# AI-Application-and-Integration-Lab/RDPN6D

Measured on AMD Instinct MI355X. Metric: RGB-D crops/sec (fwd+PnP) at 256x256, higher is better.
Workload: dtype f32

## Files before the change

include/rdpn6d.h:

```cpp
#ifndef RDPN6D_H
#define RDPN6D_H

#ifdef __cplusplus
extern "C" {
#endif

#define RDPN6D_OK 0
#define RDPN6D_EINVAL -1
#define RDPN6D_EHIP -2
#define RDPN6D_ENOMEM -3

const char* rdpn6d_last_error(void);
int rdpn6d_version(void);
int rdpn6d_device_count(void);

void farthest_point_sampling(float* pts, int* idxs, int pn, int sn);
void farthest_point_sampling_init_center(float* pts, int* idxs, int pn, int sn);
int rdpn6d_fps_host(const float* pts, int* idxs, int pn, int sn, int start);
int rdpn6d_fps_device(const float* d_pts, const int* d_offsets, int nobj, int max_pn, int sn, int start,
                      int* d_idxs, float* d_mindist, void* stream);
long long rdpn6d_fps_workspace_bytes(int nobj);
int rdpn6d_fps_device_ws(const float* d_pts, const int* d_offsets, int nobj, int max_pn, int sn, int start, int* d_idxs,
                         float* d_mindist, void* workspace, long long workspace_bytes, void* stream);

// ... 206 lines not shown
int rdpn6d_dense_glue_backward_f32(const float* head, int head_cs, const float* coord2d, const float* fps, const int* argmax,
                                   const float* dpnp, int pnp_cs, int B, int HW, int K, int mask_attention,
                                   const float* minmax, float* dhead, float* datt_scratch, void* stream);
int rdpn6d_dense_losses_mt_f32(const float* head, int head_cs, const float* gt_xyz, const float* mask_visib, const float* mask_trunc,
                               const long long* gt_region, int B, int HW, int K, float xyz_lw, float mask_lw, float region_lw,
                               int mask_type, float* dhead, float* losses, double* scratch, void* stream);
int rdpn6d_dense_glue_backward_mt_f32(const float* head, int head_cs, const float* coord2d, const float* fps, const int* argmax,
                                      const float* dpnp, int pnp_cs, int B, int HW, int K, int mask_attention, int mask_type,
                                      const float* minmax, float* dhead, float* datt_scratch, void* stream);
int rdpn6d_pose_train_f32(const float* rt, int rt_stride, const float* roi_cams, const float* roi_centers,
                          const float* roi_whs, const float* resize_ratios, const float* roi_extents, const float* gt_rot,
                          const float* gt_trans_ratio, const float* points, int npts, int B, int is_allo, float pm_lw,
                          int pm_norm_by_extent, float centroid_lw, float z_lw, float* rot, float* trans, float* d_rt,
                          float* losses, float* scratch, void* stream);
int rdpn6d_pose_train_sym_f32(const float* rt, int rt_stride, const float* roi_cams, const float* roi_centers,
                              const float* roi_whs, const float* resize_ratios, const float* roi_extents,
                              const float* gt_rot, const float* gt_trans_ratio, const float* points, int npts, int B,
                              int is_allo, float pm_lw, int pm_norm_by_extent, float centroid_lw, float z_lw,
                              const float* sym_rots, const int* sym_counts, int ksym, float* gt_rot_used, float* rot,
                              float* trans, float* d_rt, float* losses, float* scratch, void* stream);
int rdpn6d_train_vis_scalars_f32(const float* rot, const float* trans, const float* gt_rot, const float* gt_trans, const float* rt,
                                 int rt_stride, const float* gt_trans_ratio, int B, float* out17, void* stream);
int rdpn6d_ranger_step_f32(float* param, const float* grad, float* exp_avg, float* exp_avg_sq, float* slow, const void* work,
                           int nwork, const long long* row_off, const int* row_len, int nrows, float* row_mean, float beta1,
                           float beta2, float eps, float neg_step_lr, float wd_lr, int rectified, int lookahead, float alpha,
                           void* stream);
int rdpn6d_ranger_step_scaled_f32(float* param, const float* grad, float* exp_avg, float* exp_avg_sq, float* slow, const void* work,
                                  int nwork, const long long* row_off, const int* row_len, int nrows, float* row_mean, float beta1,
                                  float beta2, float eps, float neg_step_lr, float wd_lr, int rectified, int lookahead, float alpha,
                                  float inv_scale, const int* found_inf, void* stream);
int rdpn6d_grad_nonfinite_f32(const float* grad, long long n, int* flag, void* stream);
int rdpn6d_act_backward_f32(float* dy, const float* y, long long n, float slope, void* stream);
int rdpn6d_transpose_rc_f32(const float* x, int B, int R, int C, float* y, void* stream);
int rdpn6d_rgb_to_nhwc4_f32(const float* x, int B, int xc, int R, float* y, void* stream);
int rdpn6d_stem_im2col_f32(const float* x, int B, int xc, int R, float* out, void* stream);
int rdpn6d_stem_rowpatch_f32(const float* x, int B, int xc, int R, float* out, void* stream);

typedef struct {
    const float* src;
    float* dst;
    void* dst_bf16;
    const int* operm;
    const int* iperm;
    long long so, si, start;
    int O, T, I, dT, dIpad;
    int toff[9];
} rdpn6d_repack_desc;
int rdpn6d_repack_f32(const rdpn6d_repack_desc* table_dev, const int* blk_desc_dev, const long long* blk_off_dev, int nblocks,
                      void* stream);

int rdpn6d_bn_train_stats_bf16(const void* x, long long M, int C, int cs, int co, float eps, float momentum, float* mean,
                               float* invstd, float* running_mean, float* running_var, double* scratch, void* stream);
int rdpn6d_bn_apply_bf16(const void* x, int xcs, int xco, const float* mean, const float* invstd, const float* gamma,
                         const float* beta, const void* res, int rcs, int rco, void* y, int ycs, int yco, long long M, int C,
                         int relu, void* stream);
int rdpn6d_bn_backward_bf16(const void* x, int xcs, int xco, const void* dy, int dcs, int dco, const void* y, int ycs, int yco,
                            const float* mean, const float* invstd, const float* gamma, float* dgamma, float* dbeta, void* dx,
                            int xgcs, int xgco, void* dres, int rcs, int rco, long long M, int C, int relu, double* scratch,
                            void* stream);
int rdpn6d_bn_relu_backward_bf16(const void* x, int xcs, int xco, const void* dy, int dcs, int dco, const float* mean,
                                 const float* invstd, const float* gamma, const float* beta, float* dgamma, float* dbeta, void* dx,
                                 int xgcs, int xgco, long long M, int C, double* scratch, void* stream);
int rdpn6d_channel_sum_bf16(const void* x, long long M, int C, int cs, int co, float* out, int accumulate, double* scratch,
                            void* stream);
int rdpn6d_maxpool3x3s2_backward_bf16(const void* x, const void* dy, int B, int H, int W, int C, void* dx, void* stream);
int rdpn6d_upsample_bilinear_backward_bf16(const void* dy, int B, int H, int W, int C, int factor, void* dx, void* stream);
// ... 103 lines not shown
```

rdpn6d_amd/_lib.py:

```python
import ctypes
import os

HERE = os.path.dirname(os.path.abspath(__file__))
LIB_PATH = os.environ.get("RDPN6D_LIB") or os.path.join(HERE, "librdpn6d_hip.so")

_ll = ctypes.c_longlong
c_float_p = ctypes.c_void_p
c_int_p = ctypes.c_void_p
_vp, _i, _f, _u = ctypes.c_void_p, ctypes.c_int, ctypes.c_float, ctypes.c_uint


class ConvDesc(ctypes.Structure):

    _fields_ = [
        ("x", _vp), ("w", _vp), ("scale", _vp), ("shift", _vp), ("res", _vp), ("y", _vp),
        ("B", _i), ("H", _i), ("W", _i), ("Cin", _i), ("in_cs", _i), ("in_co", _i), ("Ho", _i), ("Wo", _i),
        ("stride", _i), ("ntaps", _i), ("dy", _i * 9), ("dx", _i * 9), ("N", _i), ("Npad", _i), ("OH", _i), ("OW", _i),
        ("osy", _i), ("osx", _i), ("ooy", _i), ("oox", _i), ("out_cs", _i), ("out_co", _i), ("res_cs", _i),
        ("res_co", _i), ("act", _i), ("slope", _f),
    ]


SIGNATURES = {
    "rdpn6d_last_error": (ctypes.c_char_p, []),
# ... 65 lines not shown
    "rdpn6d_groupnorm_relu_train_f32": (_i, [_vp, _vp, _i, _i, _i, _i, _vp, _vp, _vp, _vp]),
    "rdpn6d_groupnorm_relu_backward_f32": (_i, [_vp, _vp, _vp, _vp, _vp, _vp, _vp, _vp, _vp, _vp, _i, _i, _i, _i, _vp]),
    "rdpn6d_wgrad_scratch_floats": (_ll, [_i, _i, _i, _i, _i, _i]),
    "rdpn6d_wgrad_f32": (_i, [_vp, _i, _i, _i, _vp, _i, _i, _i, _i, _i, _i, _i, _i, _i, _i, _vp, _vp, _vp, _vp, _vp]),
    "rdpn6d_wgrad_bf16": (_i, [_vp, _i, _i, _i, _i, _vp, _i, _i, _i, _i, _i, _i, _i, _i, _i, _i, _i, _vp, _vp, _vp, _vp, _vp]),
    "rdpn6d_wgrad_f32_strided": (_i, [_vp, _i, _i, _i, _vp, _i, _i, _i, _i, _i, _i, _i, _i, _i, _i, _vp, _vp, _vp, _ll, _ll, _ll, _i, _i,
                                      _vp, _vp]),
    "rdpn6d_wgrad_bf16_strided": (_i, [_vp, _i, _i, _i, _i, _vp, _i, _i, _i, _i, _i, _i, _i, _i, _i, _i, _i, _vp, _vp, _vp, _ll, _ll, _ll,
                                       _i, _i, _vp, _vp]),
    "rdpn6d_wgrad_group_scratch_floats": (_ll, [_i, _i, _i, _i, _i, _i, _i]),
    "rdpn6d_wgrad_bf16_group": (_i, [_i, _vp, _i, _i, _i, _i, _vp, _i, _i, _i, _i, _i, _i, _i, _i, _i, _i, _i, _vp, _vp, _vp, _ll, _ll, _ll,
                                     _i, _i, _vp, _ll, _vp]),
    "rdpn6d_wgrad_bf16x3_strided": (_i, [_vp, _ll, _i, _i, _i, _i, _vp, _ll, _i, _i, _i, _i, _i, _i, _i, _i, _i, _i, _i, _vp, _vp, _vp,
                                         _ll, _ll, _ll, _i, _i, _vp, _vp]),
    "rdpn6d_maxpool3x3s2_backward_f32": (_i, [_vp, _vp, _i, _i, _i, _i, _vp, _vp]),
    "rdpn6d_upsample_bilinear_backward_f32": (_i, [_vp, _i, _i, _i, _i, _i, _vp, _vp]),
    "rdpn6d_global_max_concat_backward_f32": (_i, [_vp, _vp, _i, _i, _i, _i, _vp, _vp]),
    "rdpn6d_dense_losses_f32": (_i, [_vp, _i, _vp, _vp, _vp, _vp, _i, _i, _i, _f, _f, _f, _vp, _vp, _vp, _vp]),
    "rdpn6d_dense_glue_backward_f32": (_i, [_vp, _i, _vp, _vp, _vp, _vp, _i, _i, _i, _i, _i, _vp, _vp, _vp, _vp]),
    "rdpn6d_dense_losses_mt_f32": (_i, [_vp, _i, _vp, _vp, _vp, _vp, _i, _i, _i, _f, _f, _f, _i, _vp, _vp, _vp, _vp]),
    "rdpn6d_dense_glue_backward_mt_f32": (_i, [_vp, _i, _vp, _vp, _vp, _vp, _i, _i, _i, _i, _i, _i, _vp, _vp, _vp, _vp]),
    "rdpn6d_pose_train_f32": (_i, [_vp, _i, _vp, _vp, _vp, _vp, _vp, _vp, _vp, _vp, _i, _i, _i, _f, _i, _f, _f, _vp, _vp, _vp,
                                   _vp, _vp, _vp]),
    "rdpn6d_pose_train_sym_f32": (_i, [_vp, _i, _vp, _vp, _vp, _vp, _vp, _vp, _vp, _vp, _i, _i, _i, _f, _i, _f, _f, _vp, _vp, _i,
                                       _vp, _vp, _vp, _vp, _vp, _vp, _vp]),
    "rdpn6d_ranger_step_f32": (_i, [_vp, _vp, _vp, _vp, _vp, _vp, _i, _vp, _vp, _i, _vp, _f, _f, _f, _f, _f, _i, _i, _f, _vp]),
    "rdpn6d_ranger_step_scaled_f32": (_i, [_vp, _vp, _vp, _vp, _vp, _vp, _i, _vp, _vp, _i, _vp, _f, _f, _f, _f, _f, _i, _i, _f, _f, _vp, _vp]),
    "rdpn6d_grad_nonfinite_f32": (_i, [_vp, _ll, _vp, _vp]),
    "rdpn6d_region_targets_f32": (_i, [_vp, _vp, _vp, _vp, _i, _i, _i, _vp, _vp, _vp]),
    "rdpn6d_pose_errors_f64": (_i, [_vp, _vp, _vp, _i, _i, _i, _vp, _vp, _vp]),
    "rdpn6d_crop_builder_f32": (_i, [_vp, _vp, _i, _i, _i, _vp, _vp, _vp, _vp, _vp, _i, _i, _vp, _vp, _vp]),
    "rdpn6d_act_backward_f32": (_i, [_vp, _vp, _ll, _f, _vp]),
    "rdpn6d_transpose_rc_f32": (_i, [_vp, _i, _i, _i, _vp, _vp]),
    "rdpn6d_train_vis_scalars_f32": (_i, [_vp, _vp, _vp, _vp, _vp, _i, _vp, _i, _vp, _vp]),
    "rdpn6d_rgb_to_nhwc4_f32": (_i, [_vp, _i, _i, _i, _vp, _vp]),
    "rdpn6d_stem_im2col_f32": (_i, [_vp, _i, _i, _i, _vp, _vp]),
    "rdpn6d_stem_rowpatch_f32": (_i, [_vp, _i, _i, _i, _vp, _vp]),
    "rdpn6d_stem_conv7x7_raw_bf16": (_i, [_vp, _i, _i, _i, _vp, _vp, _vp]),
    "rdpn6d_bn_train_stats_bf16": (_i, [_vp, _ll, _i, _i, _i, _f, _f, _vp, _vp, _vp, _vp, _vp, _vp]),
    "rdpn6d_bn_apply_bf16": (_i, [_vp, _i, _i, _vp, _vp, _vp, _vp, _vp, _i, _i, _vp, _i, _i, _ll, _i, _i, _vp]),
    "rdpn6d_bn_backward_bf16": (_i, [_vp, _i, _i, _vp, _i, _i, _vp, _i, _i, _vp, _vp, _vp, _vp, _vp, _vp, _i, _i, _vp, _i, _i,
                                     _ll, _i, _i, _vp, _vp]),
    "rdpn6d_bn_relu_backward_bf16": (_i, [_vp, _i, _i, _vp, _i, _i, _vp, _vp, _vp, _vp, _vp, _vp, _vp, _i, _i, _ll, _i, _vp, _vp]),
    "rdpn6d_channel_sum_bf16": (_i, [_vp, _ll, _i, _i, _i, _vp, _i, _vp, _vp]),
    "rdpn6d_maxpool3x3s2_backward_bf16": (_i, [_vp, _vp, _i, _i, _i, _i, _vp, _vp]),
    "rdpn6d_upsample_bilinear_backward_bf16": (_i, [_vp, _i, _i, _i, _i, _i, _vp, _vp]),
    "rdpn6d_global_max_concat_backward_bf16": (_i, [_vp, _vp, _i, _i, _i, _i, _vp, _vp]),
    "rdpn6d_stem_im2col_bf16": (_i, [_vp, _i, _i, _i, _vp, _vp]),
    "rdpn6d_stem_rowpatch_bf16": (_i, [_vp, _i, _i, _i, _vp, _vp]),
    "rdpn6d_repack_f32": (_i, [_vp, _vp, _vp, _i, _vp]),
    "rdpn6d_split_h2": (_i, [_vp, _i, _i, _i, _vp, _ll, _vp, _vp]),
    "rdpn6d_conv_h2_kernel_for": (_i, [_vp]),
    "rdpn6d_conv2d_h2": (_i, [_vp, _vp, _vp, _vp, _vp]),
    "rdpn6d_upsample_bilinear_h2": (_i, [_vp, _i, _i, _i, _i, _i, _vp, _vp, _vp]),
    "rdpn6d_xyz_subsample_h2": (_i, [_vp, _i, _i, _i, _i, _vp, _i, _i, _vp, _vp]),
    "rdpn6d_stem_pool_h2": (_i, [_vp, _i, _i, _i, _vp, _vp, _vp, _vp, _vp, _vp]),
    "rdpn6d_stem_pool_h2_ex": (_i, [_vp, _i, _i, _i, _vp, _vp, _vp, _vp, _i, _vp, _vp]),
    "rdpn6d_stem_pack_h2": (_i, [_vp, _vp, _vp, _vp]),
    "rdpn6d_global_max_concat_h2": (_i, [_vp, _i, _i, _i, _i, _vp]),
    "rdpn6d_upsample_bilinear_h2_ex": (_i, [_vp, _i, _i, _i, _i, _i, _vp, _i, _i, _i, _vp, _vp]),
    "rdpn6d_global_max_h2": (_i, [_vp, _i, _i, _i, _i, _vp, _vp]),
    "rdpn6d_convt3x3s2_const_bias_f32": (_i, [_vp, _vp, _i, _i, _vp, _vp]),
    "rdpn6d_conv2d_h2_cb": (_i, [_vp, _vp, _vp, _vp, _vp, _vp]),
    "rdpn6d_conv2d_h2_ws": (_i, [_vp, _vp, _vp, _vp, _vp, _vp, ctypes.c_longlong, _vp]),
    "rdpn6d_conv_h2_fuse1x1_ok": (_i, [ctypes.POINTER(ConvDesc)]),
    "rdpn6d_conv2d_h2_fuse1x1": (_i, [ctypes.POINTER(ConvDesc), _vp, _vp, _vp, _vp, _vp, _vp, _vp, _i, _i, _vp]),
# ... 50 lines not shown
```

rdpn6d_amd/build.py:

```python
import os
import subprocess
import sys

HERE = os.path.dirname(os.path.abspath(__file__))
CSRC = os.path.join(HERE, "csrc")
LIB = os.path.join(HERE, "librdpn6d_hip.so")
SOURCES = ["api.cpp", "conv_igemm.hip", "conv_igemm_bf16.hip", "conv_igemm_bf16_8ph.hip", "conv_igemm_bf16_pp.hip", "conv_igemm_bf16x3.hip", "conv_igemm_bf16x3_tile.hip", "conv_igemm_h2.hip", "conv_igemm_h2_pp.hip", "pointwise.hip", "pointwise_bf16.hip", "pointwise_h2.hip", "fps.hip", "ransac.hip", "train_norm.hip", "train_wgrad.hip", "train_misc.hip", "ranger.hip", "targets_eval.hip", "crop_builder.hip", "pnp.hip"]
NO_CONTRACT = {"fps.hip", "ransac.hip", "targets_eval.hip", "crop_builder.hip", "pnp.hip"}
FLAGS = ["--offload-arch=gfx950", "-O3", "-std=c++17", "-fPIC", "-Wall", "-Wno-unused-function"]
LP_SOURCES = ["conv_igemm_bf16.hip", "conv_igemm_bf16_8ph.hip", "conv_igemm_bf16_pp.hip", "pointwise_bf16.hip", "pointwise.hip", "train_norm.hip", "train_misc.hip",
              "train_wgrad.hip"]
LP_EXTRA_RENAMES = {"rdpn6d_repack_f32": "rdpn6d_repack_fp16"}
if os.environ.get("RDPN6D_PROBE"):
    FLAGS.append("-DRDPN6D_PROBE")


def _stale():
    if not os.path.exists(LIB):
        return True
    t = os.path.getmtime(LIB)
    deps = [os.path.join(CSRC, f) for f in os.listdir(CSRC)] + [os.path.join(HERE, "..", "include", "rdpn6d.h")]
    return any(os.path.getmtime(d) > t for d in deps)


def build(force=False, verbose=True):
    if not force and not _stale():
        return LIB
    hipcc = os.environ.get("HIPCC", "/opt/rocm/bin/hipcc")
    objs = []
    os.makedirs(os.path.join(HERE, "build"), exist_ok=True)
    procs = []
    for src in SOURCES:
        obj = os.path.join(HERE, "build", src + ".o")
        objs.append(obj)
        extra = ["-ffp-contract=off"] if src in NO_CONTRACT else []
        cmd = [hipcc] + FLAGS + extra + ["-c", os.path.join(CSRC, src), "-o", obj]
        procs.append((src, subprocess.Popen(cmd, stdout=subprocess.PIPE, stderr=subprocess.STDOUT, text=True)))
    lp_objs = []
    for src in LP_SOURCES:
        obj = os.path.join(HERE, "build", "fp16_" + src + ".o")
# ... 40 lines not shown
```

rdpn6d_amd/config.py:

```python
import ast
import copy
import os


class ConfigDict(dict):

    def __init__(self, *a, **k):
        super().__init__()
        for key, v in dict(*a, **k).items():
            self[key] = v

    def __setitem__(self, k, v):
        super().__setitem__(k, _wrap(v))

    def __getattr__(self, k):
        try:
            return self[k]
        except KeyError as e:
            raise AttributeError(f"config has no key '{k}'") from e

    def __setattr__(self, k, v):
        self[k] = v

    def update(self, *a, **k):
# ... 82 lines not shown
            WEIGHTS="",
            PIXEL_MEAN=[0.0, 0.0, 0.0],
            PIXEL_STD=[255.0, 255.0, 255.0],
            CDPN=dict(
                NAME="GDRN",
                TASK="rot",
                USE_MTL=False,
                BACKBONE=dict(PRETRAINED="", ARCH="resnet", NUM_LAYERS=34, INPUT_CHANNEL=3, INPUT_RES=256,
                              OUTPUT_RES=64, FREEZE=False),
                ROT_HEAD=dict(
                    FREEZE=False, ROT_CONCAT=False, XYZ_BIN=64, NUM_LAYERS=3, NUM_FILTERS=256, CONV_KERNEL_SIZE=3,
                    NORM="BN", NUM_GN_GROUPS=32, OUT_CONV_KERNEL_SIZE=1, NUM_CLASSES=num_classes,
                    ROT_CLASS_AWARE=False, XYZ_LOSS_TYPE="L1", XYZ_LOSS_MASK_GT="visib", XYZ_LW=1.0,
                    MASK_CLASS_AWARE=False, MASK_LOSS_TYPE="L1", MASK_LOSS_GT="trunc", MASK_LW=1.0,
                    MASK_THR_TEST=0.5, NUM_REGIONS=num_regions, REGION_CLASS_AWARE=False, REGION_LOSS_TYPE="CE",
                    REGION_LOSS_MASK_GT="visib", REGION_LW=1.0,
                ),
                PNP_NET=dict(
                    FREEZE=False, R_ONLY=False, LR_MULT=1.0,
                    PNP_HEAD_CFG=dict(type="ConvPnPNet", norm="GN", num_gn_groups=32, drop_prob=0.0),
                    WITH_2D_COORD=True, REGION_ATTENTION=True, MASK_ATTENTION=mask_attention,
                    TRANS_WITH_BOX_INFO="none", ROT_TYPE="allo_rot6d", TRANS_TYPE="centroid_z", Z_TYPE="REL",
                    NUM_PM_POINTS=3000, PM_LOSS_TYPE="L1", PM_SMOOTH_L1_BETA=1.0, PM_LOSS_SYM=False,
                    PM_NORM_BY_EXTENT=True, PM_R_ONLY=True, PM_DISENTANGLE_T=False, PM_DISENTANGLE_Z=False,
                    PM_T_USE_POINTS=False, PM_LW=1.0, ROT_LOSS_TYPE="angular", ROT_LW=0.0,
                    CENTROID_LOSS_TYPE="L1", CENTROID_LW=1.0, Z_LOSS_TYPE="L1", Z_LW=1.0, TRANS_LOSS_TYPE="L1",
                    TRANS_LOSS_DISENTANGLE=True, TRANS_LW=0.0, BIND_LOSS_TYPE="L1", BIND_LW=0.0,
                ),
                TRANS_HEAD=dict(ENABLED=False, FREEZE=True, LR_MULT=1.0, NUM_LAYERS=3, NUM_FILTERS=256, NORM="BN",
                                NUM_GN_GROUPS=32, CONV_KERNEL_SIZE=3, OUT_CHANNEL=3, TRANS_TYPE="centroid_z",
                                Z_TYPE="REL"),
            ),
        ),
        SOLVER=dict(IMS_PER_BATCH=24, BASE_LR=1e-4, BF16X3=True, GROUP_WGRAD=True, OPTIMIZER_CFG=dict(type="Ranger", lr=1e-4, weight_decay=0),
                    WEIGHT_DECAY=0.0, AMP=dict(ENABLED=False, DTYPE="bf16")),
        INPUT=dict(FORMAT="BGR", DZI_PAD_SCALE=1.5),
        TRAIN=dict(VIS_SCALARS=False, VIS_PERIOD=20),
        TEST=dict(USE_PNP=False, PNP_TYPE="ransac_pnp", AMP_TEST=False, AMP_DTYPE="bf16", BF16X3=True, FP16X2=True, FOLD_GLOBAL_MAX=True, CONV_BEFORE_UPSAMPLE=True, COMPOSE_CONV3_CONVT=True, PNP_H2=True, FUSE_HEAD_OUT=True, PNP_SIDE_STREAM=True, TEST_BBOX_TYPE="est"),
    )
```

rdpn6d_amd/train.py:

```python
import ctypes
import os

import torch

from . import _lib
from .gdrn import _pad_to, _ptr

BN_EPS, BN_MOM = 1e-5, 0.1


def _taps(k, pad):
    return [(ky - pad, kx - pad) for ky in range(k) for kx in range(k)]


class TrainEngine:
    def __init__(self, model, B, device, amp=False):
        self.lib = _lib.load()
        self.model, self.B, self.dev = model, B, device
        self.amp = bool(amp)
        self.lp = "fp16" if amp == "fp16" else "bf16"
        self.lp_dtype = torch.float16 if self.lp == "fp16" else torch.bfloat16
        self.loss_scale = 1.0
        self.accumulate_grad = False
        self._seed_factor = 1.0
        self._consumed = True
        self.adt = self.lp_dtype if self.amp else torch.float32
        self.sfx = self.lp if self.amp else "f32"
        self._casts = {}
        self.mirrors = []
        self.mirrors3 = []
        self._planes = {}
        self.x3 = (not self.amp) and bool(model.cfg.get("SOLVER", {}).get("BF16X3", True))
        self.bn_fuse_stats = bool(model.cfg.get("SOLVER", {}).get("BN_FUSE_STATS", os.environ.get("RDPN6D_BN_FUSE_STATS", "1") != "0"))
        self.bn_fuse_bwd = bool(model.cfg.get("SOLVER", {}).get("BN_FUSE_BWD", os.environ.get("RDPN6D_BN_FUSE_BWD", "1") != "0"))
        self._bn_by_dy, self._scratch_bnb_need = {}, 0
        self.repack_tiles = os.environ.get("RDPN6D_REPACK_TILES", "1") != "0"
        self.bn_fuse_bwd_res = bool(model.cfg.get("SOLVER", {}).get("BN_FUSE_BWD_RES", os.environ.get("RDPN6D_BN_FUSE_BWD_RES", "1") != "0"))
        self.bn_remask = bool(model.cfg.get("SOLVER", {}).get("BN_REMASK", os.environ.get("RDPN6D_BN_REMASK", "1") != "0"))
        self.x3_launches = 0
        cfg = model.cfg
        self.R = int(cfg.MODEL.CDPN.BACKBONE.INPUT_RES)
        self.K = int(cfg.MODEL.CDPN.ROT_HEAD.NUM_REGIONS)
        pc, rc = cfg.MODEL.CDPN.PNP_NET, cfg.MODEL.CDPN.ROT_HEAD
        self.mask_attention = 1 if pc.MASK_ATTENTION == "mul" else 0
        if pc.MASK_ATTENTION not in ("none", "mul"):
            raise ValueError("MASK_ATTENTION must be none | mul")
        if rc.XYZ_LOSS_TYPE != "L1" or rc.REGION_LOSS_TYPE != "CE":
            raise NotImplementedError("only the xyz / region loss types of the shipped RGB-D configs (L1 / CE) are implemented")
        from .gdrn import MASK_TYPES

        if rc.MASK_LOSS_TYPE not in MASK_TYPES:
            raise NotImplementedError(f"unknown mask loss type: {rc.MASK_LOSS_TYPE}")
        self.mask_type = MASK_TYPES[str(rc.MASK_LOSS_TYPE)]
        if self.mask_type == 2 and self.mask_attention:
            raise NotImplementedError("MASK_ATTENTION with ROT_HEAD.MASK_LOSS_TYPE='CE': get_mask_prob's CE branch raises in the reference "
                                      "itself (torch.softmax has no keepdim argument, models/model_utils.py:39)")
        if rc.XYZ_LOSS_MASK_GT != "visib" or rc.MASK_LOSS_GT != "trunc" or rc.REGION_LOSS_MASK_GT != "visib":
            raise NotImplementedError("loss mask selection other than visib/trunc/visib is not implemented")
        if not (pc.PM_R_ONLY and pc.PM_LOSS_TYPE == "L1" and pc.PM_LW > 0):
            raise NotImplementedError("only the PM_R_ONLY L1 point-matching loss is implemented")
        self.pm_sym = bool(pc.PM_LOSS_SYM)
        if pc.CENTROID_LOSS_TYPE != "L1" or pc.Z_LOSS_TYPE != "L1" or pc.ROT_LW > 0 or pc.TRANS_LW > 0 or pc.get("BIND_LW", 0) > 0:
            raise NotImplementedError("only L1 centroid / z losses (ROT_LW = TRANS_LW = BIND_LW = 0) are implemented")
        self.lw = dict(xyz=float(rc.XYZ_LW), mask=float(rc.MASK_LW), region=float(rc.REGION_LW), pm=float(pc.PM_LW),
                       centroid=float(pc.CENTROID_LW), z=float(pc.Z_LW), pm_norm=1 if pc.PM_NORM_BY_EXTENT else 0)
        self.is_allo = 1 if "allo" in pc.ROT_TYPE else 0
        self.bufs = {}
        self._sym_cache = None
        self._bn_counters = []
        self.repack = []
        self.fwd, self.bwd = [], []
        self.records = []
# ... 817 lines not shown
                                                                               _ptr(datt), self.st()), "glue bwd")])
        self._group_marks[len(self.bwd)] = "pnp_net"
        x, d_x, hw, cin_real, cs = pnp_in, d_pnp_in, R4, 11 + K, self.pnp_cs
        for i in range(0, 9, 3):
            conv, gn = pnp.features[i], pnp.features[i + 1]
            fd = conv.weight.shape[0]
            oh = hw // 2
            r_i, a_i = self.buf(f"raw:pnp{i}", B, oh, oh, fd), self.buf(f"act:pnp{i}", B, oh, oh, fd)
            d_ri = self.conv_unit(f"pnp_net.features.{i}", conv, x, (hw, hw), cs, 0, cin_real, r_i, (oh, oh), fd, 0, stride=2, dx=d_x)
            stats = self.buf(f"gnstats:{i}", B, gn.groups, 2)
            ga, be = gn.weight, gn.bias
            self.fwd.append(lambda r_i=r_i, a_i=a_i, oh=oh, fd=fd, gn=gn, ga=ga, be=be, stats=stats: _lib.check(
                lib.rdpn6d_groupnorm_relu_train_f32(_ptr(r_i), _ptr(a_i), B, oh * oh, fd, gn.groups, _ptr(ga), _ptr(be), _ptr(stats), self.st()), "gn"))
            d_ai = self.buf(f"d:pnp_act{i}", B, oh, oh, fd, zero=True)
            dgb = self.buf(f"dgb:pnp{i}", B, 2, fd)

            def gn_bwd(r_i=r_i, a_i=a_i, d_ai=d_ai, d_ri=d_ri, oh=oh, fd=fd, gn=gn, ga=ga, stats=stats, dgb=dgb):
                _lib.check(lib.rdpn6d_groupnorm_relu_backward_f32(_ptr(r_i), _ptr(a_i), _ptr(d_ai), _ptr(ga), _ptr(stats), _ptr(d_ri),
                                                                  _ptr(self._grad(gn.weight)), _ptr(self._grad(gn.bias)), _ptr(dgb),
                                                                  _ptr(self._scratch_d), B, oh * oh, fd, gn.groups, self.st()), "gn bwd")

            self.bwd.append([gn_bwd])
            x, d_x, hw, cin_real, cs = a_i, d_ai, oh, fd, fd
        kin = cs * hw * hw
        f1, f2 = self.buf("act:fc1", B, 1024), self.buf("act:fc2", B, 256)
        self.rt = self.buf("act:rt", B, 16, zero=True)
        d_f1, d_f2 = self.buf("d:fc1", B, 1024, zero=True), self.buf("d:fc2", B, 256, zero=True)
        self.d_rt = self.buf("d:rt", B, 16, zero=True)
        x_t, d_xt = self.buf("act:pnp_flat", B, cs, hw * hw), self.buf("d:pnp_flat", B, cs, hw * hw, zero=True)
        self.fwd.append(lambda x=x, x_t=x_t: _lib.check(lib.rdpn6d_transpose_rc_f32(_ptr(x), B, hw * hw, cs, _ptr(x_t), self.st()), "flatten"))
        self.bwd.append([lambda d_x=d_x, d_xt=d_xt: _lib.check(lib.rdpn6d_transpose_rc_f32(_ptr(d_xt), B, cs, hw * hw, _ptr(d_x), self.st()),
                                                              "flatten bwd")])
        self._fc("fc1", pnp.fc1.weight, pnp.fc1.bias, x_t.view(B, kin), d_xt.view(B, kin), kin, f1, d_f1, 1024, act=2)
        self._fc("fc2", pnp.fc2.weight, pnp.fc2.bias, f1, d_f1, 1024, f2, d_f2, 256, act=2)
        self._fc("fc_rt", (pnp.fc_r.weight, pnp.fc_t.weight), (pnp.fc_r.bias, pnp.fc_t.bias), f2, d_f2, 256, self.rt, self.d_rt, 9, act=0, out_cs=16)
        self.rot, self.trans = self.buf("rot", B, 3, 3), self.buf("trans", B, 3)
        self.gt_rot_used = self.buf("gt_rot_used", B, 3, 3)
        self.losses9 = self.buf("losses", 16, zero=True)

    def _fc(self, name, w, b, x, d_x, kin, y, d_y, nout, act, out_cs=None, w_view=None, g_view=None):
        lib, B = self.lib, self.B
        ws = w if isinstance(w, tuple) else (w,)
        bs = b if isinstance(b, tuple) else (b,)
        out_cs = out_cs or nout
        npad = _pad_to(nout, 64)

        k_perm = None
        if w_view is not None:
            k_perm = w_view(torch.arange(kin, dtype=torch.float32).view(1, kin))[0].long().tolist()
        wf = torch.zeros(npad, 1, kin, dtype=torch.float32, device=self.dev)
        bvec = torch.zeros(npad, dtype=torch.float32, device=self.dev)
        r0 = 0
        for wp_, bp_ in zip(ws, bs):
            n = wp_.shape[0]
            self._pack_map(None, wp_, n, 1, kin, kin, 1, [0], iperm=k_perm, dst=wf, dst_off=r0 * kin, dT=1, dIpad=kin)
            self._pack_map(None, bp_, 1, 1, n, 0, 1, [0], dst=bvec, dst_off=r0, dT=1, dIpad=npad)
            r0 += n
        d = self._conv_desc(x, (1, 1), kin, 0, kin, wf, y, (1, 1), out_cs, 0, nout, [(0, 0)], shift=bvec, act=act, slope=0.1)
        self.fwd.append(self._launch_conv(name, d, (wf, bvec), ksplit=True))
        ca = _pad_to(nout, 4)
        wg_out = self.buf("wg:" + name, ca, 1, kin)
        self._wg_floats = max(self._wg_floats, int(lib.rdpn6d_wgrad_scratch_floats(B, 1, 1, ca, kin, 1)))
        z9 = (ctypes.c_int * 9)(*([0] * 9))
        bg = self.buf("bg:" + name, npad)
        n_red = _pad_to(nout, 16)
        assert out_cs >= n_red
        wd = torch.zeros(_pad_to(kin, 64), 1, n_red, dtype=torch.float32, device=self.dev)
        r0 = 0
        for wp_ in ws:
            n = wp_.shape[0]
            self._pack_map(None, wp_, kin, 1, n, 1, kin, [0], operm=k_perm, dst=wd, dst_off=r0, dT=1, dIpad=n_red)
            r0 += n
        dd = self._conv_desc(d_y, (1, 1), out_cs, 0, n_red, wd, d_x, (1, 1), kin, 0, kin, [(0, 0)])

        def bwd():
            if act == 2:
                _lib.check(lib.rdpn6d_act_backward_f32(_ptr(d_y), _ptr(y), B * out_cs, 0.1, self.st()), "leaky bwd " + name)
# ... 173 lines not shown
```

Measured before the change: 9297.

## Add small-batch FC kernels for the PnP head instead of 1x1 conv path

Adds dedicated forward, dgrad and wgrad kernels for fully connected layers with small batch (B<=64). They read the weights in place instead of packing them, use split-K over kin with a separate reduce, and fuse the leaky-ReLU backward into dgrad. The change targets the PnP head's fc1/fc2/fc_rt, which previously ran as 1x1 implicit-GEMM convolutions that are poorly shaped for M=24. The cost is extra workspace and a second reduce launch, plus an error raised at run time if a weight or gradient is not contiguous.

```diff
diff --git a/include/rdpn6d.h b/include/rdpn6d.h
--- a/include/rdpn6d.h
+++ b/include/rdpn6d.h
@@ -262,6 +262,13 @@
 int rdpn6d_grad_nonfinite_f32(const float* grad, long long n, int* flag, void* stream);
 int rdpn6d_act_backward_f32(float* dy, const float* y, long long n, float slope, void* stream);
 int rdpn6d_transpose_rc_f32(const float* x, int B, int R, int C, float* y, void* stream);
+long long rdpn6d_fc_forward_ws_floats(int B, int kin, int nout);
+int rdpn6d_fc_forward_f32(const float* x, int B, int kin, const float* const* w, const float* const* bias, const int* rows, int nparams,
+                          int nout, float* y, int y_stride, int act, float slope, float* ws, long long ws_floats, void* stream);
+int rdpn6d_fc_dgrad_f32(const float* dy, int dy_stride, int B, int kin, const float* const* w, const int* rows, int nparams, int nout,
+                        const float* x_act, float slope, float* dx, void* stream);
+int rdpn6d_fc_wgrad_f32(const float* dy, int dy_stride, const float* x, int B, int kin, float* const* gw, float* const* gb,
+                        const int* rows, int nparams, int nout, void* stream);
 int rdpn6d_rgb_to_nhwc4_f32(const float* x, int B, int xc, int R, float* y, void* stream);
 int rdpn6d_stem_im2col_f32(const float* x, int B, int xc, int R, float* out, void* stream);
 int rdpn6d_stem_rowpatch_f32(const float* x, int B, int xc, int R, float* out, void* stream);
diff --git a/rdpn6d_amd/_lib.py b/rdpn6d_amd/_lib.py
--- a/rdpn6d_amd/_lib.py
+++ b/rdpn6d_amd/_lib.py
@@ -121,6 +121,10 @@
     "rdpn6d_crop_builder_f32": (_i, [_vp, _vp, _i, _i, _i, _vp, _vp, _vp, _vp, _vp, _i, _i, _vp, _vp, _vp]),
     "rdpn6d_act_backward_f32": (_i, [_vp, _vp, _ll, _f, _vp]),
     "rdpn6d_transpose_rc_f32": (_i, [_vp, _i, _i, _i, _vp, _vp]),
+    "rdpn6d_fc_forward_ws_floats": (_ll, [_i, _i, _i]),
+    "rdpn6d_fc_forward_f32": (_i, [_vp, _i, _i, _vp, _vp, _vp, _i, _i, _vp, _i, _i, _f, _vp, _ll, _vp]),
+    "rdpn6d_fc_dgrad_f32": (_i, [_vp, _i, _i, _i, _vp, _vp, _i, _i, _vp, _f, _vp, _vp]),
+    "rdpn6d_fc_wgrad_f32": (_i, [_vp, _i, _vp, _i, _i, _vp, _vp, _vp, _i, _i, _vp]),
     "rdpn6d_train_vis_scalars_f32": (_i, [_vp, _vp, _vp, _vp, _vp, _i, _vp, _i, _vp, _vp]),
     "rdpn6d_rgb_to_nhwc4_f32": (_i, [_vp, _i, _i, _i, _vp, _vp]),
     "rdpn6d_stem_im2col_f32": (_i, [_vp, _i, _i, _i, _vp, _vp]),
diff --git a/rdpn6d_amd/build.py b/rdpn6d_amd/build.py
--- a/rdpn6d_amd/build.py
+++ b/rdpn6d_amd/build.py
@@ -5,7 +5,7 @@
 HERE = os.path.dirname(os.path.abspath(__file__))
 CSRC = os.path.join(HERE, "csrc")
 LIB = os.path.join(HERE, "librdpn6d_hip.so")
-SOURCES = ["api.cpp", "conv_igemm.hip", "conv_igemm_bf16.hip", "conv_igemm_bf16_8ph.hip", "conv_igemm_bf16_pp.hip", "conv_igemm_bf16x3.hip", "conv_igemm_bf16x3_tile.hip", "conv_igemm_h2.hip", "conv_igemm_h2_pp.hip", "pointwise.hip", "pointwise_bf16.hip", "pointwise_h2.hip", "fps.hip", "ransac.hip", "train_norm.hip", "train_wgrad.hip", "train_misc.hip", "ranger.hip", "targets_eval.hip", "crop_builder.hip", "pnp.hip"]
+SOURCES = ["api.cpp", "conv_igemm.hip", "conv_igemm_bf16.hip", "conv_igemm_bf16_8ph.hip", "conv_igemm_bf16_pp.hip", "conv_igemm_bf16x3.hip", "conv_igemm_bf16x3_tile.hip", "conv_igemm_h2.hip", "conv_igemm_h2_pp.hip", "pointwise.hip", "pointwise_bf16.hip", "pointwise_h2.hip", "fps.hip", "ransac.hip", "train_norm.hip", "train_wgrad.hip", "train_misc.hip", "fc_small_m.hip", "ranger.hip", "targets_eval.hip", "crop_builder.hip", "pnp.hip"]
 NO_CONTRACT = {"fps.hip", "ransac.hip", "targets_eval.hip", "crop_builder.hip", "pnp.hip"}
 FLAGS = ["--offload-arch=gfx950", "-O3", "-std=c++17", "-fPIC", "-Wall", "-Wno-unused-function"]
 LP_SOURCES = ["conv_igemm_bf16.hip", "conv_igemm_bf16_8ph.hip", "conv_igemm_bf16_pp.hip", "pointwise_bf16.hip", "pointwise.hip", "train_norm.hip", "train_misc.hip",
diff --git a/rdpn6d_amd/config.py b/rdpn6d_amd/config.py
--- a/rdpn6d_amd/config.py
+++ b/rdpn6d_amd/config.py
@@ -138,7 +138,7 @@
                                 Z_TYPE="REL"),
             ),
         ),
-        SOLVER=dict(IMS_PER_BATCH=24, BASE_LR=1e-4, BF16X3=True, GROUP_WGRAD=True, OPTIMIZER_CFG=dict(type="Ranger", lr=1e-4, weight_decay=0),
+        SOLVER=dict(IMS_PER_BATCH=24, BASE_LR=1e-4, BF16X3=True, GROUP_WGRAD=True, FC_SMALL_M=True, OPTIMIZER_CFG=dict(type="Ranger", lr=1e-4, weight_decay=0),
                     WEIGHT_DECAY=0.0, AMP=dict(ENABLED=False, DTYPE="bf16")),
         INPUT=dict(FORMAT="BGR", DZI_PAD_SCALE=1.5),
         TRAIN=dict(VIS_SCALARS=False, VIS_PERIOD=20),
diff --git a/rdpn6d_amd/csrc/fc_small_m.hip b/rdpn6d_amd/csrc/fc_small_m.hip
--- /dev/null
+++ b/rdpn6d_amd/csrc/fc_small_m.hip
@@ -0,0 +1,388 @@
+#include "common.h"
+
+#define FC_MAXP 4
+
+struct FcParams {
+    const float* w[FC_MAXP];
+    const float* b[FC_MAXP];
+    float* gw[FC_MAXP];
+    float* gb[FC_MAXP];
+    int row0[FC_MAXP];
+    int n;
+};
+
+__device__ __forceinline__ int fc_param_of(const FcParams& p, int n, int& local)
+{
+    int which = 0;
+    local = n;
+#pragma unroll
+    for (int i = 1; i < FC_MAXP; ++i)
+        if (i < p.n && n >= p.row0[i]) {
+            which = i;
+            local = n - p.row0[i];
+        }
+    return which;
+}
+#define FC_PICK(arr, which) ((which) == 0 ? (arr)[0] : (which) == 1 ? (arr)[1] : (which) == 2 ? (arr)[2] : (arr)[3])
+
+__device__ __forceinline__ const float* fc_w_row(const FcParams& p, int n, int kin)
+{
+    int local;
+    const int which = fc_param_of(p, n, local);
+    return FC_PICK(p.w, which) + (long long)local * kin;
+}
+
+#define FCF_ROWS 16
+#define FCF_STEP 256
+
+template <int H> __device__ __forceinline__ void fc_fold(float (&v)[128], int lane)
+{
+    const bool up = (lane & (H / 2)) != 0;
+#pragma unroll
+    for (int j = 0; j < H; ++j) {
+        const float send = up ? v[j] : v[j + H];
+        const float keep = up ? v[j + H] : v[j];
+        v[j] = keep + __shfl_xor(send, H / 2);
+    }
+}
+
+__global__ __launch_bounds__(256) void fc_fwd_partial_kernel(const float* __restrict__ x, int B, int kin, FcParams p, int nout, int steps_per,
+                                                             float* __restrict__ part, int npad)
+{
+    __shared__ f32x4 xs[32 * 64];
+    const int tid = threadIdx.x, lane = tid & 63, wave = __builtin_amdgcn_readfirstlane(tid >> 6);
+    const int n0 = blockIdx.x * FCF_ROWS + wave * 4;
+    const int s = blockIdx.y, S = gridDim.y, b0 = blockIdx.z * 32;
+    const int kbeg = s * steps_per * FCF_STEP;
+    const float* wr[4];
+#pragma unroll
+    for (int r = 0; r < 4; ++r) wr[r] = fc_w_row(p, min(n0 + r, nout - 1), kin);
+    float v[128];
+#pragma unroll
+    for (int i = 0; i < 128; ++i) v[i] = 0.f;
+    f32x4 xn[8];
+    float wn[4][4];
+    auto load_step = [&](int k0) {
+#pragma unroll
+        for (int i = 0; i < 8; ++i) {
+            const int idx = i * 256 + tid, b = idx >> 6, c = idx & 63;
+            xn[i] = f32x4{0.f, 0.f, 0.f, 0.f};
+            if (b0 + b < B && k0 + c * 4 < kin) xn[i] = *reinterpret_cast<const f32x4*>(x + (long long)(b0 + b) * kin + k0 + c * 4);
+        }
+#pragma unroll
+        for (int r = 0; r < 4; ++r)
+#pragma unroll
+            for (int j = 0; j < 4; ++j) {
+                const int k = k0 + j * 64 + lane;
+                wn[r][j] = k < kin ? wr[r][k] : 0.f;
+            }
+    };
+    load_step(kbeg);
+    for (int step = 0; step < steps_per; ++step) {
+        const int k0 = kbeg + step * FCF_STEP;
+        if (k0 >= kin) break;
+        __syncthreads();
+#pragma unroll
+        for (int i = 0; i < 8; ++i) xs[i * 256 + tid] = xn[i];
+        float w4[4][4];
+#pragma unroll
+        for (int r = 0; r < 4; ++r)
+#pragma unroll
+            for (int j = 0; j < 4; ++j) w4[r][j] = wn[r][j];
+        __syncthreads();
+        if (step + 1 < steps_per && k0 + FCF_STEP < kin) load_step(k0 + FCF_STEP);
+        const float* xsf = reinterpret_cast<const float*>(xs);
+#pragma unroll
+        for (int b = 0; b < 32; ++b) {
+            float xv[4];
+#pragma unroll
+            for (int j = 0; j < 4; ++j) xv[j] = xsf[b * 256 + j * 64 + lane];
+#pragma unroll
+            for (int r = 0; r < 4; ++r) {
+                float a = v[r * 32 + b];
+                a = __builtin_fmaf(w4[r][0], xv[0], a);
+                a = __builtin_fmaf(w4[r][1], xv[1], a);
+                a = __builtin_fmaf(w4[r][2], xv[2], a);
+                a = __builtin_fmaf(w4[r][3], xv[3], a);
+                v[r * 32 + b] = a;
+            }
+        }
+    }
+    fc_fold<64>(v, lane);
+    fc_fold<32>(v, lane);
+    fc_fold<16>(v, lane);
+    fc_fold<8>(v, lane);
+    fc_fold<4>(v, lane);
+    fc_fold<2>(v, lane);
+    const int n = n0 + (lane >> 4), b = (lane & 15) * 2;
+    float* dst = part + (((long long)blockIdx.z * S + s) * npad + n) * 32 + b;
+    *reinterpret_cast<float2*>(dst) = make_float2(v[0], v[1]);
+}
+
+__global__ __launch_bounds__(256) void fc_fwd_reduce_kernel(const float* __restrict__ part, int S, int npad, FcParams p, int B, int nout,
+                                                            float* __restrict__ y, int y_stride, int act, float slope)
+{
+    const int i = blockIdx.x * 256 + threadIdx.x;
+    if (i >= B * nout) return;
+    const int b = i % B, n = i / B;
+    const float* src = part + ((long long)(b >> 5) * S * npad + n) * 32 + (b & 31);
+    float a = 0.f;
+    for (int s = 0; s < S; ++s) a += src[(long long)s * npad * 32];
+    int local;
+    const int which = fc_param_of(p, n, local);
+    const float* bias = FC_PICK(p.b, which);
+    if (bias) a += bias[local];
+    if (act == 1) a = a > 0.f ? a : 0.f;
+    else if (act == 2) a = a > 0.f ? a : a * slope;
+    y[(long long)b * y_stride + n] = a;
+}
+
+static void fc_fwd_plan(int kin, int nout, int& ntiles, int& S, int& steps_per)
+{
+    ntiles = rd_cdiv(nout, FCF_ROWS);
+    const int steps = rd_cdiv(kin, FCF_STEP);
+    int want = 512 / ntiles;
+    if (want < 1) want = 1;
+    if (want > steps) want = steps;
+    steps_per = rd_cdiv(steps, want);
+    S = rd_cdiv(steps, steps_per);
+}
+
+static int fc_fill(FcParams& p, const float* const* w, const float* const* bias, float* const* gw, float* const* gb, const int* rows,
+                   int nparams, int nout)
+{
+    memset(&p, 0, sizeof(p));
+    RD_REQUIRE(rows && nparams >= 1 && nparams <= FC_MAXP, "1..4 parameters behind one activation");
+    int r0 = 0;
+    for (int i = 0; i < nparams; ++i) {
+        RD_REQUIRE(rows[i] > 0, "rows of a parameter");
+        if (w) {
+            RD_REQUIRE(w[i], "weight pointer");
+            p.w[i] = w[i];
+        }
+        if (bias) p.b[i] = bias[i];
+        if (gw) {
+            RD_REQUIRE(gw[i], "weight gradient pointer");
+            p.gw[i] = gw[i];
+        }
+        if (gb) p.gb[i] = gb[i];
+        p.row0[i] = r0;
+        r0 += rows[i];
+    }
+    RD_REQUIRE(r0 == nout, "the parameters' rows add up to nout");
+    p.n = nparams;
+    return RDPN6D_OK;
+}
+
+#define FC_SHAPE_CHECK()                                                                                              \
+    RD_REQUIRE(B >= 1 && B <= 64, "rows B in 1..64 (larger batches run as 1x1 convolutions)");                        \
+    RD_REQUIRE(kin >= 4 && kin % 4 == 0 && nout >= 1 && nout <= (1 << 20) && kin <= (1 << 24), "kin a multiple of 4")
+
+extern "C" long long rdpn6d_fc_forward_ws_floats(int B, int kin, int nout)
+{
+    if (B < 1 || B > 64 || kin < 4 || nout < 1) return 0;
+    int ntiles, S, steps_per;
+    fc_fwd_plan(kin, nout, ntiles, S, steps_per);
+    return (long long)((B + 31) / 32) * S * ntiles * FCF_ROWS * 32;
+}
+
+extern "C" int rdpn6d_fc_forward_f32(const float* x, int B, int kin, const float* const* w, const float* const* bias, const int* rows,
+                                     int nparams, int nout, float* y, int y_stride, int act, float slope, float* ws, long long ws_floats,
+                                     void* stream)
+{
+    FC_SHAPE_CHECK();
+    RD_REQUIRE(x && w && y && ws && ((size_t)x & 15) == 0 && ((size_t)ws & 15) == 0, "null / unaligned pointer");
+    RD_REQUIRE(y_stride >= nout && act >= 0 && act <= 2, "output stride / activation");
+    FcParams p;
+    if (int rc = fc_fill(p, w, bias, nullptr, nullptr, rows, nparams, nout)) return rc;
+    int ntiles, S, steps_per;
+    fc_fwd_plan(kin, nout, ntiles, S, steps_per);
+    RD_REQUIRE(ws_floats >= rdpn6d_fc_forward_ws_floats(B, kin, nout), "workspace too small");
+    const int npad = ntiles * FCF_ROWS;
+    hipLaunchKernelGGL(fc_fwd_partial_kernel, dim3(ntiles, S, (B + 31) / 32), dim3(256), 0, (hipStream_t)stream, x, B, kin, p, nout, steps_per,
+                       ws, npad);
+    RD_LAUNCH_CHECK();
+    hipLaunchKernelGGL(fc_fwd_reduce_kernel, dim3(rd_cdiv((long)B * nout, 256)), dim3(256), 0, (hipStream_t)stream, ws, S, npad, p, B, nout, y,
+                       y_stride, act, slope);
+    RD_LAUNCH_CHECK();
+    return RDPN6D_OK;
+}
+
+#define FCD_COLS 64
+#define FCD_BT 16
+#define FCD_NC 512
+
+__global__ __launch_bounds__(512) void fc_dgrad_kernel(const float* __restrict__ dy, int dy_stride, int B, int nout, int kin, FcParams p,
+                                                       const float* __restrict__ xact, float slope, float* __restrict__ dx)
+{
+    __shared__ f32x4 sm[FCD_NC * 4];
+    const int tid = threadIdx.x, lane = tid & 63, wave = __builtin_amdgcn_readfirstlane(tid >> 6);
+    const int col = blockIdx.x * FCD_COLS + lane, colc = min(col, kin - 1);
+    const int b0 = blockIdx.y * FCD_BT;
+    float acc[FCD_BT];
+#pragma unroll
+    for (int i = 0; i < FCD_BT; ++i) acc[i] = 0.f;
+    for (int nc = 0; nc < nout; nc += FCD_NC) {
+        const unsigned long long myrow = (unsigned long long)(fc_w_row(p, min(nc + lane * 8 + wave, nout - 1), kin) - p.w[0]);
+        const unsigned row_lo = (unsigned)myrow, row_hi = (unsigned)(myrow >> 32);
+        float wv[FCD_NC / 8];
+#pragma unroll
+        for (int i = 0; i < FCD_NC / 8; ++i) {
+            wv[i] = 0.f;
+            if (nc + i * 8 < nout) {
+                const unsigned long long rp = ((unsigned long long)__builtin_amdgcn_readlane(row_hi, i) << 32) | __builtin_amdgcn_readlane(row_lo, i);
+                wv[i] = (p.w[0] + (long long)rp)[colc];
+            }
+        }
+        __syncthreads();
+        {
+            const int n = nc + tid;
+            float t[FCD_BT];
+#pragma unroll
+            for (int i = 0; i < FCD_BT; ++i) t[i] = (n < nout && b0 + i < B) ? dy[(long long)(b0 + i) * dy_stride + n] : 0.f;
+#pragma unroll
+            for (int q = 0; q < 4; ++q) sm[tid * 4 + q] = f32x4{t[4 * q], t[4 * q + 1], t[4 * q + 2], t[4 * q + 3]};
+        }
+        __syncthreads();
+#pragma unroll
+        for (int i = 0; i < FCD_NC / 8; ++i) {
+            if (nc + i * 8 < nout) {
+#pragma unroll
+                for (int q = 0; q < 4; ++q) {
+                    const f32x4 d = sm[(i * 8 + wave) * 4 + q];
+#pragma unroll
+                    for (int j = 0; j < 4; ++j) acc[4 * q + j] = __builtin_fmaf(d[j], wv[i], acc[4 * q + j]);
+                }
+            }
+        }
+    }
+    __syncthreads();
+    float* red = reinterpret_cast<float*>(sm);
+#pragma unroll
+    for (int i = 0; i < FCD_BT; ++i) red[(wave * FCD_BT + i) * 64 + lane] = acc[i];
+    __syncthreads();
+#pragma unroll
+    for (int o = tid; o < FCD_BT * 64; o += 512) {
+        const int i = o >> 6, c = o & 63;
+        double sd = 0.0;
+#pragma unroll
+        for (int w = 0; w < 8; ++w) sd += (double)red[(w * FCD_BT + i) * 64 + c];
+        float s = (float)sd;
+        const int b = b0 + i, k = blockIdx.x * FCD_COLS + c;
+        if (b < B && k < kin) {
+            if (xact) s = xact[(long long)b * kin + k] > 0.f ? s : s * slope;
+            dx[(long long)b * kin + k] = s;
+        }
+    }
+}
+
+extern "C" int rdpn6d_fc_dgrad_f32(const float* dy, int dy_stride, int B, int kin, const float* const* w, const int* rows, int nparams,
+                                   int nout, const float* x_act, float slope, float* dx, void* stream)
+{
+    FC_SHAPE_CHECK();
+    RD_REQUIRE(dy && w && dx && dy_stride >= nout, "null pointer / stride");
+    FcParams p;
+    if (int rc = fc_fill(p, w, nullptr, nullptr, nullptr, rows, nparams, nout)) return rc;
+    hipLaunchKernelGGL(fc_dgrad_kernel, dim3(rd_cdiv(kin, FCD_COLS), rd_cdiv(B, FCD_BT)), dim3(512), 0, (hipStream_t)stream, dy, dy_stride, B,
+                       nout, kin, p, x_act, slope, dx);
+    RD_LAUNCH_CHECK();
+    return RDPN6D_OK;
+}
+
+#ifndef FCW_RPW
+#define FCW_RPW 16
+#endif
+#define FCW_ROWS (4 * FCW_RPW)
+#define FCW_COLS 256
+#define FCW_BT 16
+#ifndef FCW_OCC
+#define FCW_OCC 2
+#endif
+
+__global__ __launch_bounds__(256, FCW_OCC) void fc_wgrad_kernel(const float* __restrict__ dy, int dy_stride, const float* __restrict__ x, int B, int nout,
+                                                       int kin, FcParams p)
+{
+    __shared__ f32x4 sm[FCW_ROWS * 4];
+    const int tid = threadIdx.x, lane = tid & 63, wave = __builtin_amdgcn_readfirstlane(tid >> 6);
+    const int k = blockIdx.x * FCW_COLS + lane;
+    const int nb = blockIdx.y * FCW_ROWS, nw = nb + wave * FCW_RPW;
+    float acc[FCW_RPW][4];
+#pragma unroll
+    for (int r = 0; r < FCW_RPW; ++r)
+#pragma unroll
+        for (int j = 0; j < 4; ++j) acc[r][j] = 0.f;
+    float gbias = 0.f;
+    int kc[4];
+#pragma unroll
+    for (int j = 0; j < 4; ++j) kc[j] = min(k + 64 * j, kin - 1);
+    for (int b0 = 0; b0 < B; b0 += FCW_BT) {
+        float xr[FCW_BT][4];
+#pragma unroll
+        for (int b = 0; b < FCW_BT; ++b)
+#pragma unroll
+            for (int j = 0; j < 4; ++j) {
+                const float* xrow = x + (long long)min(b0 + b, B - 1) * kin;
+                const float t = xrow[kc[j]];
+                xr[b][j] = b0 + b < B ? t : 0.f;
+            }
+        __syncthreads();
+        {
+            const int row = tid % FCW_ROWS, bq = tid / FCW_ROWS, n = nb + row;
+            float t[4];
+#pragma unroll
+            for (int i = 0; i < 4; ++i) {
+                const int b = b0 + bq * 4 + i;
+                t[i] = (n < nout && b < B) ? dy[(long long)b * dy_stride + n] : 0.f;
+            }
+            sm[row * 4 + bq] = f32x4{t[0], t[1], t[2], t[3]};
+        }
+        __syncthreads();
+#pragma unroll
+        for (int r = 0; r < FCW_RPW; ++r) {
+#pragma unroll
+            for (int q = 0; q < 4; ++q) {
+                const f32x4 d = sm[(wave * FCW_RPW + r) * 4 + q];
+#pragma unroll
+                for (int i = 0; i < 4; ++i)
+#pragma unroll
+                    for (int j = 0; j < 4; ++j) acc[r][j] = __builtin_fmaf(d[i], xr[4 * q + i][j], acc[r][j]);
+            }
+            asm volatile("" : "+v"(acc[r][0]), "+v"(acc[r][1]), "+v"(acc[r][2]), "+v"(acc[r][3])::"memory");
+        }
+        if (blockIdx.x == 0 && tid < FCW_ROWS) {
+            const float* row = reinterpret_cast<const float*>(sm) + tid * FCW_BT;
+            for (int b = 0; b < FCW_BT; ++b) gbias += row[b];
+        }
+    }
+#pragma unroll
+    for (int r = 0; r < FCW_RPW; ++r) {
+        const int n = nw + r;
+        if (n < nout) {
+            int local;
+            const int which = fc_param_of(p, n, local);
+            float* g = FC_PICK(p.gw, which) + (long long)local * kin + k;
+#pragma unroll
+            for (int j = 0; j < 4; ++j)
+                if (k + 64 * j < kin) g[64 * j] = acc[r][j];
+        }
+    }
+    if (blockIdx.x == 0 && tid < FCW_ROWS && nb + tid < nout) {
+        int local;
+        const int which = fc_param_of(p, nb + tid, local);
+        float* g = FC_PICK(p.gb, which);
+        if (g) g[local] = gbias;
+    }
+}
+
+extern "C" int rdpn6d_fc_wgrad_f32(const float* dy, int dy_stride, const float* x, int B, int kin, float* const* gw, float* const* gb,
+                                   const int* rows, int nparams, int nout, void* stream)
+{
+    FC_SHAPE_CHECK();
+    RD_REQUIRE(dy && x && gw && dy_stride >= nout, "null pointer / stride");
+    FcParams p;
+    if (int rc = fc_fill(p, nullptr, nullptr, gw, gb, rows, nparams, nout)) return rc;
+    hipLaunchKernelGGL(fc_wgrad_kernel, dim3(rd_cdiv(kin, FCW_COLS), rd_cdiv(nout, FCW_ROWS)), dim3(256), 0, (hipStream_t)stream, dy, dy_stride,
+                       x, B, nout, kin, p);
+    RD_LAUNCH_CHECK();
+    return RDPN6D_OK;
+}
diff --git a/rdpn6d_amd/train.py b/rdpn6d_amd/train.py
--- a/rdpn6d_amd/train.py
+++ b/rdpn6d_amd/train.py
@@ -38,6 +38,8 @@
         self.bn_fuse_bwd_res = bool(model.cfg.get("SOLVER", {}).get("BN_FUSE_BWD_RES", os.environ.get("RDPN6D_BN_FUSE_BWD_RES", "1") != "0"))
         self.bn_remask = bool(model.cfg.get("SOLVER", {}).get("BN_REMASK", os.environ.get("RDPN6D_BN_REMASK", "1") != "0"))
         self.x3_launches = 0
+        self.fc_small_m = (bool(model.cfg.get("SOLVER", {}).get("FC_SMALL_M", True)) and os.environ.get("RDPN6D_FC_SMALL_M", "1") != "0"
+                           and B <= 64)
         cfg = model.cfg
         self.R = int(cfg.MODEL.CDPN.BACKBONE.INPUT_RES)
         self.K = int(cfg.MODEL.CDPN.ROT_HEAD.NUM_REGIONS)
@@ -921,17 +923,48 @@
         self.bwd.append([lambda d_x=d_x, d_xt=d_xt: _lib.check(lib.rdpn6d_transpose_rc_f32(_ptr(d_xt), B, cs, hw * hw, _ptr(d_x), self.st()),
                                                               "flatten bwd")])
         self._fc("fc1", pnp.fc1.weight, pnp.fc1.bias, x_t.view(B, kin), d_xt.view(B, kin), kin, f1, d_f1, 1024, act=2)
-        self._fc("fc2", pnp.fc2.weight, pnp.fc2.bias, f1, d_f1, 1024, f2, d_f2, 256, act=2)
-        self._fc("fc_rt", (pnp.fc_r.weight, pnp.fc_t.weight), (pnp.fc_r.bias, pnp.fc_t.bias), f2, d_f2, 256, self.rt, self.d_rt, 9, act=0, out_cs=16)
+        self._fc("fc2", pnp.fc2.weight, pnp.fc2.bias, f1, d_f1, 1024, f2, d_f2, 256, act=2, x_act=2)
+        self._fc("fc_rt", (pnp.fc_r.weight, pnp.fc_t.weight), (pnp.fc_r.bias, pnp.fc_t.bias), f2, d_f2, 256, self.rt, self.d_rt, 9, act=0, out_cs=16,
+                 x_act=2)
         self.rot, self.trans = self.buf("rot", B, 3, 3), self.buf("trans", B, 3)
         self.gt_rot_used = self.buf("gt_rot_used", B, 3, 3)
         self.losses9 = self.buf("losses", 16, zero=True)
 
-    def _fc(self, name, w, b, x, d_x, kin, y, d_y, nout, act, out_cs=None, w_view=None, g_view=None):
+    def _fc_small_m(self, name, ws, bs, x, d_x, kin, y, d_y, nout, act, out_cs, x_act):
+        lib, B = self.lib, self.B
+        n = len(ws)
+        rows = (ctypes.c_int * n)(*[int(wp.shape[0]) for wp in ws])
+        assert all(tuple(wp.shape) == (r, kin) and wp.dtype == torch.float32 for wp, r in zip(ws, rows)) and sum(rows) == nout
+        ptrs = lambda ts: (ctypes.c_void_p * n)(*[t.data_ptr() for t in ts])
+        ws_n = int(lib.rdpn6d_fc_forward_ws_floats(B, kin, nout))
+        wsb = self.buf("fc_ws:" + name, ws_n)
+
+        def fwd():
+            for wp in ws:
+                if not wp.is_contiguous():
+                    raise RuntimeError(f"{name}: a weight that is not contiguous cannot be read in place (cfg.SOLVER.FC_SMALL_M)")
+            _lib.check(lib.rdpn6d_fc_forward_f32(_ptr(x), B, kin, ptrs(ws), ptrs(bs), rows, n, nout, _ptr(y), out_cs, act, 0.1, _ptr(wsb),
+                                                 ws_n, self.st()), name)
+
+        def bwd():
+            gws, gbs = [self._grad(wp) for wp in ws], [self._grad(bp) for bp in bs]
+            if not all(g.is_contiguous() for g in gws + gbs):
+                raise RuntimeError(f"{name}: a gradient that is not contiguous cannot be written in place (cfg.SOLVER.FC_SMALL_M)")
+            _lib.check(lib.rdpn6d_fc_wgrad_f32(_ptr(d_y), out_cs, _ptr(x), B, kin, ptrs(gws), ptrs(gbs), rows, n, nout, self.st()),
+                       "wgrad " + name)
+            _lib.check(lib.rdpn6d_fc_dgrad_f32(_ptr(d_y), out_cs, B, kin, ptrs(ws), rows, n, nout, _ptr(x) if x_act == 2 else None, 0.1,
+                                               _ptr(d_x), self.st()), "dgrad " + name)
+
+        self.fwd.append(fwd)
+        self.bwd.append([bwd])
+
+    def _fc(self, name, w, b, x, d_x, kin, y, d_y, nout, act, out_cs=None, w_view=None, g_view=None, x_act=0):
         lib, B = self.lib, self.B
         ws = w if isinstance(w, tuple) else (w,)
         bs = b if isinstance(b, tuple) else (b,)
         out_cs = out_cs or nout
+        if self.fc_small_m and w_view is None and g_view is None:
+            return self._fc_small_m(name, ws, bs, x, d_x, kin, y, d_y, nout, act, out_cs, x_act)
         npad = _pad_to(nout, 64)
 
         k_perm = None
```

Measured after the change: 9283. Within noise of the previous version (-0.2%).
